# bottledspace/refraction-raytracing-dxr

Hardware: AMD Instinct MI355X
Metric: Mrays/s (primary+refracted) at 1920x1080, monkey.obj (higher is better)
Workload: dtype f32

## Files before the change

refraction_raytracing_dxr_amd/_build.py:

```python
import os
import shutil
import subprocess

PKG = os.path.dirname(os.path.abspath(__file__))
CSRC = os.path.join(PKG, "csrc")
LIB = os.path.join(PKG, "librrdxr.so")
DEMO = os.path.join(PKG, "rrdemo")

DEVICE_SOURCES = ["rr_bvh_build.hip", "rr_render_fused.hip", "rr_render_paths.hip", "rr_render_lds.hip", "rr_render_stream.hip",
                  "rr_query.hip", "rr_query_multi.hip", "rr_frame.hip", "rr_shade_rays.hip", "rr_render_samples.hip",
                  "rr_render_adaptive.hip", "rr_render_lens.hip", "rr_render_spectral.hip", "rr_render_materials.hip"]
HOST_SOURCES = ["rr_capi.cpp", "rr_capi_build.cpp", "rr_capi_dispatch.cpp", "rr_capi_orbit.cpp", "rr_capi_query.cpp", "rr_capi_comm.cpp",
                "rr_choice.cpp", "host/rr_host_camera.cpp", "host/rr_host_mesh.cpp", "host/rr_host_image.cpp", "host/rr_host_partition.cpp",
                "host/Mesh.cpp", "host/RefractionDemo.cpp"]
HEADERS = ["rr_types.h", "rr_context.h", "rr_choice.h", "rr_device.h", "rr_launch.h", "rr_render_common.h", "rr_render_materials.h", "host/Mesh.hpp", "host/RefractionDemo.hpp", "host/rr_host_lens.h",
           "../../include/rrdxr.h"]

COMMON = ["-O3", "-std=c++17", "-fPIC", "-ffp-contract=off", "-fno-fast-math", "-Wall", "-Wno-unused-function"]
DEVICE_FLAGS = ["--offload-arch=gfx950", "-fno-gpu-rdc"] + os.environ.get("RR_EXTRA_DEFINES", "").split()


def _hipcc():
    exe = shutil.which("hipcc") or "/opt/rocm/bin/hipcc"
    if not os.path.exists(exe):
        raise RuntimeError("hipcc not found: the HIP extension cannot be built")
    return exe


def _stale(target, deps):
    if not os.path.exists(target):
        return True
    t = os.path.getmtime(target)
    return any((not os.path.exists(d)) or os.path.getmtime(d) > t for d in deps)


def build(force=False, verbose=False):
    hipcc = _hipcc()
    srcs = [os.path.join(CSRC, s) for s in DEVICE_SOURCES + HOST_SOURCES]
    deps = srcs + [os.path.join(CSRC, h) for h in HEADERS] + [os.path.abspath(__file__)]
    objdir = os.path.join(PKG, "build")
    os.makedirs(objdir, exist_ok=True)
    stamp = os.path.join(objdir, "flags.txt")
    flags = " ".join(COMMON + DEVICE_FLAGS + DEVICE_SOURCES)
    if not os.path.exists(stamp) or open(stamp).read() != flags:
        force = True
    objs = []
    for s in srcs:
        o = os.path.join(objdir, os.path.basename(s) + ".o")
        objs.append(o)
        if force or _stale(o, [s] + deps[len(srcs):]):
            cmd = [hipcc, "-c", "-x", "hip", s, "-o", o] + COMMON + DEVICE_FLAGS
            if verbose:
                print(" ".join(cmd))
            subprocess.run(cmd, check=True)
    if force or _stale(LIB, objs):
        cmd = [hipcc, "-shared", "-o", LIB] + objs + ["--offload-arch=gfx950", "-fno-gpu-rdc"]
        if verbose:
            print(" ".join(cmd))
        subprocess.run(cmd, check=True)
    if force:
        with open(stamp, "w") as f:
            f.write(flags)
    demo_src = os.path.join(CSRC, "tools", "rrdemo.cpp")
    if force or _stale(DEMO, [demo_src, LIB]):
        cmd = [hipcc, demo_src, "-o", DEMO, "-O2", "-std=c++17", "-L" + PKG, "-lrrdxr", "-Wl,-rpath,$ORIGIN"]
        subprocess.run(cmd, check=True)
    return LIB


if __name__ == "__main__":
    print(build(force=False, verbose=True))
```

refraction_raytracing_dxr_amd/csrc/rr_capi.cpp:

```cpp
#include "rr_context.h"

#include <dlfcn.h>
#include <new>

static_assert(CHOICE_TILE == (uint32_t)TILE && CHOICE_STREAM_MAX_GEN == STREAM_MAX_GEN, "rr_choice.h mirrors rr_types.h");

static_assert(sizeof(rr_vertex) == 32, "Vertex stride (Mesh.cpp:45)");
static_assert(sizeof(rr_instance_desc) == 64, "D3D12_RAYTRACING_INSTANCE_DESC");
static_assert(sizeof(rr_scene_constants) == 80, "SceneConstants");
static_assert(sizeof(rr_ray) == sizeof(rr_ray_dev) && sizeof(rr_hit) == sizeof(rr_hit_dev), "ray/hit ABI");
static_assert(offsetof(rr_ray, instance_mask) == 36 && offsetof(rr_ray_dev, instance_mask) == 36, "rr_ray.instance_mask");

namespace {
struct Roctx {
    int (*push)(const char*) = nullptr;
    int (*pop)() = nullptr;
    Roctx()
    {
        for (const char* lib : { "librocprofiler-sdk-roctx.so", "libroctx64.so" }) {
            if (void* h = dlopen(lib, RTLD_LAZY | RTLD_LOCAL)) {
                push = reinterpret_cast<int (*)(const char*)>(dlsym(h, "roctxRangePushA"));
                pop = reinterpret_cast<int (*)()>(dlsym(h, "roctxRangePop"));
                if (push && pop) return;
                push = nullptr; pop = nullptr;
// ... 51 lines not shown

uint32_t scene_stack_need(const rr_context* ctx)
{
    uint32_t blas_max = 0;
    for (uint32_t i = 0; i < ctx->n_insts; ++i) {
        const MeshRes& m = ctx->meshes[(size_t)ctx->inst_host[i].blas];
        if (m.depth > blas_max) blas_max = m.depth;
    }
    return ctx->single_identity ? blas_max : blas_max + ctx->tlas_depth;
}

Tiles tile_counts(uint32_t W, uint32_t H, uint32_t rank, uint32_t world)
{
    const uint32_t tiles_x = (W + TILE - 1) / TILE, n_tiles = tiles_x * ((H + TILE - 1) / TILE);
    return { tiles_x, n_tiles, n_tiles > rank ? (n_tiles - rank + world - 1) / world : 0, (n_tiles + world - 1) / world };
}

int join_lane(rr_context* ctx, uint32_t lane)
{
    if (ctx->lane_busy[lane]) {
        RR_HIP(hipStreamWaitEvent(ctx->stream, ctx->lane_done[lane].get(), 0));
        ctx->lane_busy[lane] = false;
    }
    return RR_OK;
}

int join_lanes(rr_context* ctx)
{
    for (uint32_t l = 0; l < rr_context::MAX_LANES; ++l)
        if (int r = join_lane(ctx, l)) return r;
    return RR_OK;
}

rr_dispatch_params params_or_default(const rr_dispatch_params* params)
{
    rr_dispatch_params p;
    return params ? *params : (rr_default_dispatch_params(&p), p);
}
}

extern "C" {
uint32_t rr_abi_version(void) { return RRDXR_ABI_VERSION; }

void rr_default_dispatch_params(rr_dispatch_params* p)
{
    if (!p) return;
    p->max_refract = 5;
    p->max_reflect = 2;
    p->ior = 1.3f;
    p->tmin_primary = 0.0001f;
    p->tmax_primary = 100.0f;
    p->tmin_secondary = 0.001f;
    p->tmax_secondary = 1000.0f;
    p->flags = 0;
}

int rr_create(int device_ordinal, rr_context** out)
{
    if (!out) return RR_ERR_INVALID_ARGUMENT;
    *out = nullptr;
    int n = 0;
    if (hipGetDeviceCount(&n) != hipSuccess || n <= 0) return RR_ERR_NO_DEVICE;
    if (device_ordinal < 0 || device_ordinal >= n) return RR_ERR_INVALID_ARGUMENT;
    hipDeviceProp_t prop;
    if (hipGetDeviceProperties(&prop, device_ordinal) != hipSuccess) return RR_ERR_NO_DEVICE;
    if (strncmp(prop.gcnArchName, "gfx950", 6) != 0) return RR_ERR_NO_DEVICE;
    rr_context* ctx = new (std::nothrow) rr_context();
    if (!ctx) return RR_ERR_OUT_OF_MEMORY;
    ctx->device = device_ordinal;
    ctx->n_cus = prop.multiProcessorCount > 0 ? prop.multiProcessorCount : 256;
    if (hipSetDevice(device_ordinal) != hipSuccess || ctx->own_stream.create(hipStreamNonBlocking) != hipSuccess ||
        ctx->d_cnt.alloc(1) != hipSuccess || ctx->d_tickets.alloc((rr_context::MAX_LANES + 1) * LDS_TICKET_WORDS) != hipSuccess) {
        delete ctx;
        return RR_ERR_DEVICE;
    }
    ctx->stream = ctx->own_stream.get();
    (void)hipMemsetAsync(ctx->d_cnt.get(), 0, sizeof(CounterBlock), ctx->stream);
    (void)hipMemsetAsync(ctx->d_tickets.get(), 0, (rr_context::MAX_LANES + 1) * LDS_TICKET_WORDS * sizeof(uint32_t), ctx->stream);
    if (const char* e = getenv("RR_DEBUG_KERNEL"))
        ctx->dbg.kernel = !strcmp(e, "fused") ? 1 : !strcmp(e, "lds") ? 4 : !strcmp(e, "paths") ? 5 : !strcmp(e, "stream") ? 10 : 0;
    if (const char* e = getenv("RR_DEBUG_STACK")) ctx->dbg.stack = atoi(e);
    if (const char* e = getenv("RR_DEBUG_TICKET")) ctx->dbg_ticket_blocks = atoi(e);
    if (const char* e = getenv("RR_DEBUG_SHAPE")) ctx->dbg_shape = atoi(e);
    if (const char* e = getenv("RR_DEBUG_REFINE_GROUPS")) ctx->dbg_refine_groups = std::max(atoi(e), 0);
    if (const char* e = getenv("RR_DEBUG_TLAS32")) ctx->dbg.tlas32 = atoi(e) != 0;
    if (const char* e = getenv("RR_DEBUG_TILE_ORDER")) ctx->dbg_tile_order = atoi(e) != 0;
    if (const char* e = getenv("RR_DEBUG_ASYNC")) { unsigned l = 2, sh = 2; if (sscanf(e, "%u,%u", &l, &sh) == 2 && l >= 1 && sh >= 1) { ctx->dbg_async[0] = l; ctx->dbg_async[1] = sh; ctx->dbg_async_set = true; } }
    if (const char* e = getenv("RR_DEBUG_DIAG")) ctx->dbg_diag = e;
    if (const char* e = getenv("RR_DEBUG_GROUP_TRACE")) ctx->dbg_group_trace = atoi(e) != 0;
    *out = ctx;
    return RR_OK;
}

int rr_destroy(rr_context* ctx)
{
    if (!ctx) return RR_ERR_INVALID_ARGUMENT;
    (void)hipSetDevice(ctx->device);
    (void)hipStreamSynchronize(ctx->stream);
    for (const Stream& s : ctx->lane_stream) if (s.get()) (void)hipStreamSynchronize(s.get());
    delete ctx;
    return RR_OK;
}

const char* rr_last_error(const rr_context* ctx) { return ctx ? ctx->err.c_str() : "null context"; }

int rr_set_stream(rr_context* ctx, void* hip_stream)
{
    if (int r = use_device(ctx)) return r;
    RR_HIP(hipStreamSynchronize(ctx->stream));
    ctx->stream = (hipStream_t)hip_stream;
    return RR_OK;
}

int rr_reset_stream(rr_context* ctx)
{
    if (int r = use_device(ctx)) return r;
    RR_HIP(hipStreamSynchronize(ctx->stream));
    ctx->stream = ctx->own_stream.get();
    return RR_OK;
}

int rr_wait(rr_context* ctx)
{
    if (int r = use_device(ctx)) return r;
    if (int r = join_lanes(ctx)) return r;
    RR_HIP(hipStreamSynchronize(ctx->stream));
    return RR_OK;
}

int rr_set_frames_in_flight(rr_context* ctx, uint32_t n)
{
    if (int r = use_device(ctx)) return r;
    if (n == 0 || n > rr_context::MAX_LANES) return fail(ctx, RR_ERR_INVALID_ARGUMENT, "rr_set_frames_in_flight: 1..4");
    ctx->frames_in_flight = n;
    return RR_OK;
}

int rr_lane_join(rr_context* ctx, uint32_t lane)
{
    if (int r = use_device(ctx)) return r;
    if (lane >= rr_context::MAX_LANES) return fail(ctx, RR_ERR_INVALID_ARGUMENT, "rr_lane_join: lane out of range");
    return join_lane(ctx, lane);
}

int rr_upload_mesh(rr_context* ctx, const rr_vertex* verts, uint32_t n_verts, const uint32_t* indices, uint32_t n_indices,
                   uint32_t* mesh_id)
{
    if (int r = use_device(ctx)) return r;
    if (!verts || !indices || !mesh_id || n_verts == 0 || n_indices < 3 || n_indices % 3 != 0)
        return fail(ctx, RR_ERR_INVALID_ARGUMENT, "rr_upload_mesh: need >= 1 triangle, n_indices % 3 == 0");
    for (uint32_t i = 0; i < n_indices; ++i)
        if (indices[i] >= n_verts) return fail(ctx, RR_ERR_INVALID_ARGUMENT, "rr_upload_mesh: index out of range");
    if (rr_host_validate_positions(verts, n_verts, nullptr) != RR_OK)
        return fail(ctx, RR_ERR_INVALID_ARGUMENT, "rr_upload_mesh: non-finite or huge (> 1e18) vertex position");
    MeshRes m;
    m.n_verts = n_verts; m.n_idx = n_indices; m.n_tris = n_indices / 3;
    RR_HIP(m.d_verts.alloc((size_t)n_verts * 8));
    if (hipError_t e = m.d_idx.alloc(n_indices)) return fail(ctx, RR_ERR_OUT_OF_MEMORY, "hipMalloc(indices)", e);
    RR_HIP_MSG(hipMemcpyAsync(m.d_verts.get(), verts, (size_t)n_verts * sizeof(rr_vertex), hipMemcpyHostToDevice, ctx->stream), "mesh upload");
    RR_HIP_MSG(hipMemcpyAsync(m.d_idx.get(), indices, (size_t)n_indices * 4, hipMemcpyHostToDevice, ctx->stream), "mesh upload");
    RR_HIP_MSG(hipStreamSynchronize(ctx->stream), "mesh upload");
    ctx->meshes.push_back(std::move(m));
    *mesh_id = (uint32_t)ctx->meshes.size() - 1u;
    return RR_OK;
}

// ... 189 lines not shown
```

refraction_raytracing_dxr_amd/csrc/rr_capi_dispatch.cpp:

```cpp
#include "rr_context.h"

namespace {
int ensure_cams(rr_context* ctx, size_t n)
{
    return n <= ctx->d_cams.size() ? RR_OK : ctx->d_cams.grow(ctx, n < 64 ? 64 : n);
}

constexpr size_t STREAM_BUDGET_MAX = (size_t)48 << 30, STREAM_BUDGET_MIN = (size_t)1 << 30;
constexpr uint32_t STREAM_BLK = 1024;

size_t stream_budget(rr_context* ctx)
{
    if (ctx->strm_budget == 0) {
        size_t free_b = 0, total_b = 0;
        size_t b = STREAM_BUDGET_MAX;
        if (hipMemGetInfo(&free_b, &total_b) == hipSuccess) b = std::min(b, free_b / 6u);
        if (const char* e = getenv("RR_DEBUG_STREAM_BUDGET_GB")) { const long g = atol(e); if (g > 0 && g <= 200) b = (size_t)g << 30; }
        ctx->strm_budget = std::max(b, STREAM_BUDGET_MIN);
    }
    return ctx->strm_budget;
}

uint32_t lds_node_bytes(const MeshRes& m) { return m.n_nodes() * (uint32_t)sizeof(QNode); }

// ... 103 lines not shown
    o.want_f32 = (p.flags & RR_DISPATCH_FLOAT_OUTPUT) != 0;
    o.compact = ctx->tile_world > 1 || ext_tiles != nullptr;
    o.rgb8 = (p.flags & RR_DISPATCH_TILES_RGB8) != 0;
    if (o.rgb8 && !ext_tiles) return fail(ctx, RR_ERR_UNSUPPORTED, "dispatch: RGB8 tiles only exist in external tile buffers (rr_render_orbit_sharded)");
    o.slice_elems = o.compact ? (size_t)o.max_local * TILE * TILE * (o.rgb8 ? 3 : 4) / 4 : (size_t)width * height;
    o.stride = ext_tiles ? req.ext_stride_elems : o.slice_elems;
    if (ext_tiles && o.want_f32) return fail(ctx, RR_ERR_UNSUPPORTED, "dispatch: float output is not available for external tile buffers");
    o.out_base = ext_tiles ? 0 : o.slice_elems * req.out_slot_depth * req.out_slot;
    if (!ext_tiles)
        if (int r = ensure_frame_buffers(ctx, o.out_base + o.slice_elems * depth, o.want_f32)) return r;
    if (width != ctx->screen_w || height != ctx->screen_h) {
        RR_HIP(hipDeviceSynchronize());
        ctx->screen_w = ctx->screen_h = 0;
        RR_HIP(ctx->d_screen.alloc((size_t)width + height));
        RR_HIP(launch_screen_tables(ctx->d_screen.get(), width, height, ctx->stream));
        RR_HIP(hipStreamSynchronize(ctx->stream));
        ctx->screen_w = width; ctx->screen_h = height;
    }
    return RR_OK;
}

void set_rect_tiles(DispatchDev& a, uint32_t x0, uint32_t y0, uint32_t w, uint32_t h)
{
    a.rt_x0 = x0; a.rt_y0 = y0; a.rt_w = w; a.rt_h = h;
    a.rt_div_w = (uint32_t)(0x100000000ull / w) + 1u;
    a.rt_div_o = a.tiles_x > w ? (uint32_t)(0x100000000ull / (a.tiles_x - w)) + 1u : 0u;
}

void point_counters(DispatchDev& a, CounterBlock* c) { a.counters = c->counters; a.ray_shards = c->shards; a.error_flag = &c->error; }

DispatchDev make_dispatch(const rr_context* ctx, const DispatchRequest& req, const Layout& o)
{
    const uint32_t width = req.width, height = req.height, depth = req.depth;
    const rr_dispatch_params& p = req.params; const MeshOut* const mesh = req.mesh;
    DispatchDev a;
    memset(&a, 0, sizeof a);
    a.sx = ctx->d_screen.get(); a.sy = ctx->d_screen.get() + width;
    a.async_leaf_num = ctx->dbg_async[0]; a.async_shade_num = ctx->dbg_async[1];
    a.group_trace = ctx->dbg_group_trace ? 1u : 0u;
    uint32_t hr[4];
    (void)rr_host_screen_rect(ctx->scene_bounds, (p.flags & RR_DISPATCH_DEBUG_NO_CULL) ? nullptr : req.h_cams, depth, width, height, hr);
    a.hx0 = hr[0]; a.hy0 = hr[1]; a.hx1 = hr[2]; a.hy1 = hr[3];
    a.W = width; a.H = height; a.tiles_x = o.tiles_x; a.n_tiles = o.n_tiles;
    if (mesh) {
        a.mesh_part = 1u; a.n_mesh_local = o.n_mesh_local; a.n_rect_tiles = o.part.n_mesh_tiles; a.mesh_rounds = o.part.rank0_rounds;
        a.out_bg = mesh->bg; a.bg_stride = mesh->bg_stride_elems;
        if (o.part.rect_w) set_rect_tiles(a, o.part.rect_x0, o.part.rect_y0, o.part.rect_w, o.part.rect_h);
    } else if (ctx->dbg_tile_order && ctx->tile_world == 1 && o.n_tiles < 65536u && a.hx1 > a.hx0 && a.hy1 > a.hy0) {
        const uint32_t tiles_y = (height + TILE - 1) / TILE;
        const uint32_t x0 = a.hx0 / TILE, y0 = a.hy0 / TILE;
        const uint32_t x1 = std::min(o.tiles_x, (a.hx1 + TILE - 1) / TILE), y1 = std::min(tiles_y, (a.hy1 + TILE - 1) / TILE);
        if (x1 > x0 && y1 > y0 && (x1 - x0) * (y1 - y0) < o.n_tiles) set_rect_tiles(a, x0, y0, x1 - x0, y1 - y0);
    }
    a.cams = req.d_cams; a.n_frames = depth;
    a.blocks_per_frame = ((o.local + 7u) & ~7u) * 4u;
    a.frame_stride = o.stride;
    a.tile_rank = ctx->tile_rank; a.tile_world = ctx->tile_world; a.n_local_tiles = o.local;
    a.n_blocks = a.blocks_per_frame * depth;
    a.compact_out = o.compact ? (o.rgb8 ? 2u : 1u) : 0u;
    a.tonemap = (p.flags & RR_DISPATCH_TONEMAP_REINHARD) ? 1u : 0u;
    a.max_refract = p.max_refract; a.max_reflect = p.max_reflect;
    a.ior = p.ior; a.inv_ior = inv_ior_of(p.ior);
    a.tmin_p = p.tmin_primary; a.tmax_p = p.tmax_primary; a.tmin_s = p.tmin_secondary; a.tmax_s = p.tmax_secondary;
    a.out_rgba8 = req.ext_tiles ? req.ext_tiles : ctx->d_rgba8.get() + o.out_base;
    a.out_f32 = o.want_f32 ? ctx->d_f32.get() + o.out_base : nullptr;
    point_counters(a, ctx->d_cnt.get());
    return a;
}

struct Launch {
    SceneDev sc;
    DispatchDev a;
    uint32_t need;
    const rr_scene_constants* h_cams; const rr_dispatch_params* p;
    FusedVariant fused;
};

int ensure_lds_park(rr_context* ctx, uint32_t slot, int max_reflect)
{
    const size_t park_need = (size_t)ctx->n_cus * 32 * (max_reflect <= 2 ? 2u : 8u) * 8 * 64;
    return ctx->d_park[slot].size() < park_need ? ctx->d_park[slot].grow(ctx, park_need) : RR_OK;
}

int launch_lds(rr_context* ctx, const Launch& L, bool stats)
{
    const MeshRes& m0 = ctx->meshes[(size_t)ctx->inst_host[0].blas];
    LdsDispatch q;
    memset(&q, 0, sizeof q);
    const uint32_t slot = stream_slot(ctx);
    q.tickets = ctx->d_tickets.get() + (size_t)slot * LDS_TICKET_WORDS;
    q.park_slots = L.p->max_reflect <= 2 ? 2u : 8u;
    if (int r = ensure_lds_park(ctx, slot, L.p->max_reflect)) return r;
    q.park = ctx->d_park[slot].get();
    uint32_t rect[4];
    (void)rr_host_screen_rect(m0.bounds, ((ctx->dbg_ticket_blocks & 3) == 1 || (L.p->flags & RR_DISPATCH_DEBUG_NO_CULL)) ? nullptr : L.h_cams, L.a.n_frames,
                     L.a.W, L.a.H, rect);
    if ((ctx->dbg_ticket_blocks & 3) == 2) rect[2] = rect[0];
    q.n_queues = (ctx->dbg_ticket_blocks & 64) ? 64u : (ctx->dbg_ticket_blocks & 128) ? LDS_QUEUES : 8u;
    q.home_xcc = (ctx->dbg_ticket_blocks & 16) ? 0u : 1u;
    q.rx0 = rect[0]; q.ry0 = rect[1]; q.rx1 = rect[2]; q.ry1 = rect[3];
    q.node_bytes = lds_node_bytes(m0);
    q.stack_entries = L.need + 1;
    RR_HIP(launch_render_lds(L.sc, L.a, q, ctx->n_cus, stats, ctx->stream, ctx->dbg_shape));
    return RR_OK;
}

int launch_kernel(rr_context* ctx, const Launch& L, int kernel, bool stats)
{
    if (kernel == K_STREAM) return render_stream(ctx, L.sc, L.a, L.a.n_frames, (int)L.need, stats);
    if (kernel == K_LDS) return launch_lds(ctx, L, stats);
    if (kernel == K_PATHS) RR_HIP(launch_render_paths(L.sc, L.a, (int)L.need, stats, ctx->stream));
    else RR_HIP(launch_render_fused(L.sc, L.a, L.fused.stack, L.fused.pend, stats, ctx->stream, L.fused.stack16));
    return RR_OK;
}

int time_candidates(rr_context* ctx, Launch L, int cand_a, int cand_b, float ms[2])
{
    if (cand_b == K_STREAM) if (int r = ensure_stream_buffers(ctx, stream_plan(ctx, L.a, L.a.n_frames))) return r;
    if (cand_a == K_LDS || cand_b == K_LDS) if (int r = ensure_lds_park(ctx, stream_slot(ctx), L.p->max_reflect)) return r;
    for (Event& e : ctx->ch_ev) if (!e.get()) RR_HIP(e.create(hipEventDefault));
    if (!ctx->d_cnt_trial.get()) RR_HIP(ctx->d_cnt_trial.alloc(1));
    RR_HIP(hipDeviceSynchronize());
    RR_HIP(hipMemsetAsync(ctx->d_cnt_trial.get(), 0, sizeof(CounterBlock), ctx->stream));
    point_counters(L.a, ctx->d_cnt_trial.get());
    if (int r = launch_kernel(ctx, L, cand_a, false)) return r;
    for (int c = 0; c < 2; ++c) {
        RR_HIP(hipEventRecord(ctx->ch_ev[2 * c].get(), ctx->stream));
        if (int r = launch_kernel(ctx, L, c == 0 ? cand_a : cand_b, false)) return r;
        RR_HIP(hipEventRecord(ctx->ch_ev[2 * c + 1].get(), ctx->stream));
    }
    RR_HIP(hipEventSynchronize(ctx->ch_ev[3].get()));
    RR_HIP(hipEventElapsedTime(&ms[0], ctx->ch_ev[0].get(), ctx->ch_ev[1].get()));
    RR_HIP(hipEventElapsedTime(&ms[1], ctx->ch_ev[2].get(), ctx->ch_ev[3].get()));
    return RR_OK;
}

int choose_kernel(rr_context* ctx, const Launch& L, const KernelPick& pk, const LaunchFacts& lf, int& kernel)
{
    kernel = pk.kernel;
    if (pk.cls == CLS_NONE) return RR_OK;
    KernelChoice* const ch = ctx->ch[pk.cls].find(choice_key(L.a.W, L.a.H, *L.p, L.a.n_frames));
    if (measure_due(*ch, lf.rect_share, lf.no_cull)) {
        float ms[2] = { 0.0f, 0.0f };
        if (int r = time_candidates(ctx, L, pk.cand_a, pk.cand_b, ms)) return r;
        record_timings(*ch, ms[0], ms[1], lf.rect_share);
        if (getenv("RR_DEBUG_CHOICE"))
            fprintf(stderr, "[rr] kernel choice: depth %u candidate %d: default %.3f ms, candidate %.3f ms (%.3f)%s\n", L.a.n_frames, pk.cand_b, ms[0], ms[1],
                    ms[1] / ms[0], ch->choice == 2 ? " -> candidate" : ch->choice == 1 ? " -> default" : " (once more)");
    }
    kernel = chosen_kernel(pk, ch, lf.rect_share);
    return RR_OK;
}
}

namespace rr {
int ensure_frame_buffers(rr_context* ctx, size_t elems, bool want_f32)
{
    if (elems > ctx->d_rgba8.size())
        if (int r = ctx->d_rgba8.grow(ctx, elems)) return r;
    if (want_f32 && elems > ctx->d_f32.size()) return ctx->d_f32.grow(ctx, elems);
    return RR_OK;
}

int check_shading_params(rr_context* ctx, const char* who, const rr_dispatch_params& p)
{
    const std::string w(who);
    if (p.max_refract < 0 || p.max_refract > 65535 || p.max_reflect < 0)
        return fail(ctx, RR_ERR_INVALID_ARGUMENT, (w + ": negative bounce limit").c_str());
    if (p.max_reflect > 8) return fail(ctx, RR_ERR_UNSUPPORTED, (w + ": max_reflect > 8 (parked-ray registers)").c_str());
    if (!(p.ior > 0.0f)) return fail(ctx, RR_ERR_INVALID_ARGUMENT, (w + ": ior must be > 0").c_str());
    return RR_OK;
}

SceneFacts scene_facts(const rr_context* ctx)
{
    SceneFacts s = { ctx->single_identity, scene_stack_need(ctx), 0, ctx->n_pool_nodes, ctx->n_pool_tris + ctx->n_insts, false };
    if (ctx->single_identity && !ctx->inst_host.empty()) {
        const MeshRes& m0 = ctx->meshes[(size_t)ctx->inst_host[0].blas];
        s.blas_tris = m0.n_tris;
        s.lds_fits = ctx->dbg.stack == 0 && m0.n_tris < 32768u && lds_kernel_shape(lds_node_bytes(m0), s.need + 1, nullptr, ctx->dbg_shape) >= 0;
    }
    return s;
}

LaunchPick pick_launch(const rr_context* ctx, const DispatchRequest& req, const uint32_t rect[4], bool compact)
{
// ... 163 lines not shown
```

refraction_raytracing_dxr_amd/csrc/rr_context.h:

```cpp
#pragma once
#include "../../include/rrdxr.h"

#include <hip/hip_runtime.h>

#include <algorithm>
#include <cmath>
#include <cstdio>
#include <cstdlib>
#include <cstring>
#include <string>
#include <vector>

#include "rr_choice.h"
#include "rr_launch.h"

namespace rr {

struct Range {
    explicit Range(const char* name);
    ~Range();
};

template <class T, bool Pinned = false> class Buf {
public:
// ... 79 lines not shown
    DevBuf<uint8_t>  pending;
};

}

using namespace rr;

struct rr_context {
    int device = 0;
    int n_cus = 256;
    Stream      own_stream;
    hipStream_t stream = nullptr;
    std::string err;

    std::vector<MeshRes> meshes;

    DevBuf<float4> d_env;
    int env_w = 0, env_h = 0;

    std::vector<rr_instance_desc> inst_host;
    DevBuf<InstDev> d_insts;
    DevBuf<BvhNode> d_pool_nodes;
    DevBuf<QNode>   d_pool_qnodes;
    QGrid    scene_grid = { { 0, 0, 0 }, { 1, 1, 1 } };
    DevBuf<TriRec>  d_pool_tris;
    DevBuf<NrmRec>  d_pool_nrms;
    uint32_t n_pool_tris = 0, n_pool_nodes = 0;
    uint32_t n_insts = 0, tlas_depth = 0;
    bool tlas_built = false;
    bool single_identity = false;
    float scene_scale = 1.0f;
    float scene_bounds[6] = { 0, 0, 0, 0, 0, 0 };
    std::vector<uint32_t> pool_node_off, pool_tri_off;
    std::vector<uint64_t> pool_version;
    DevBuf<int32_t>  d_tlas_links;
    DevBuf<uint32_t> d_tlas_visit;
    bool tlas_refittable = false;

    DevBuf<float> d_screen;
    uint32_t screen_w = 0, screen_h = 0;

    rr_scene_constants cam;
    bool cam_set = false;
    DevBuf<CamDev> d_cams;
    static constexpr int CAM_SLOTS = 4;
    HostBuf<CamDev> h_cams[CAM_SLOTS];
    Event      h_cams_ev[CAM_SLOTS];
    bool       h_cams_busy[CAM_SLOTS] = {};
    uint32_t   h_cams_next = 0;

    uint32_t tile_rank = 0, tile_world = 1;

    static constexpr uint32_t MAX_LANES = 4;
    Stream      lane_stream[MAX_LANES];
    Event       lane_fork[MAX_LANES], lane_done[MAX_LANES];
    DevBuf<CamDev> lane_cams[MAX_LANES];
    bool        lane_busy[MAX_LANES] = {};
    uint32_t    frames_in_flight = 2;
    size_t      frame_base = 0;

    uint32_t W = 0, H = 0, frame_world = 0, frame_depth = 1;
    DevBuf<uint32_t> d_rgba8;
    DevBuf<float4>   d_f32;
    DevBuf<uint32_t> d_assembled;
    bool      have_f32 = false, have_frame = false, have_assembled = false;
    uint64_t  last_pixels = 0;
    uint64_t  accum_pixels = 0;
    bool      last_stats = false;

    DevBuf<CounterBlock> d_cnt;
    DevBuf<CounterBlock> d_cnt_trial;
    DevBuf<uint32_t> d_park[MAX_LANES + 1];
    char       last_kernel_name[96] = "";
    uint32_t   last_kernel = 0;
    DevBuf<uint32_t> d_tickets;

    DebugFacts dbg = { 0, 0, false };
    int  dbg_ticket_blocks = 0;
    bool dbg_group_trace = true;
    bool dbg_async_set = false;
    uint32_t dbg_async[2] = { 2, 2 };
    bool dbg_tile_order = true;
    int  dbg_shape = 0;
    int  dbg_refine_groups = 0;
    std::string dbg_diag;

    Event ev_begin, ev_end;
    std::vector<Event> kev;
    uint32_t kev_used = 0;

    StreamSet strm[MAX_LANES + 1];
    size_t    strm_budget = 0;
    ChoiceClass ch[3];
    Event      ch_ev[4];

    DevBuf<rr_ray_dev> d_rays;
    DevBuf<rr_hit_dev> d_hits;
    DevBuf<uint32_t>   d_counts;
    DevBuf<float4>     d_out_f32;
    DevBuf<uint32_t>   d_out_rgba8, d_out_n;
    DevBuf<uint32_t>   d_adaptive_taken;
    DevBuf<float4>     d_adaptive_ws;
    DevBuf<MatDev>     d_mats;
    uint32_t n_mats = 0, max_material = 0;
};

namespace rr {

int fail(rr_context* ctx, int code, const char* what, hipError_t e = hipSuccess);

#define RR_HIP(call)                                                                      \
    do {                                                                                  \
        hipError_t e_ = (call);                                                           \
        if (e_ != hipSuccess) return fail(ctx, e_ == hipErrorOutOfMemory ? RR_ERR_OUT_OF_MEMORY : RR_ERR_DEVICE, #call, e_); \
    } while (0)

#define RR_HIP_MSG(call, what)                                                            \
    do {                                                                                  \
        hipError_t e_ = (call);                                                           \
        if (e_ != hipSuccess) return fail(ctx, RR_ERR_DEVICE, what, e_);                  \
    } while (0)

template <class T, bool Pinned> int Buf<T, Pinned>::grow(rr_context* ctx, size_t n)
{
    RR_HIP(hipStreamSynchronize(ctx->stream));
    RR_HIP(alloc(n));
    return RR_OK;
}

int use_device(rr_context* ctx);
void fill_scene(const rr_context* ctx, SceneDev& sc);
uint32_t inst0_mask(const rr_context* ctx);
uint32_t scene_stack_need(const rr_context* ctx);
rr_dispatch_params params_or_default(const rr_dispatch_params* params);
struct Tiles { uint32_t tiles_x, n_tiles, local, max_local; };
Tiles tile_counts(uint32_t W, uint32_t H, uint32_t rank, uint32_t world);
int join_lane(rr_context* ctx, uint32_t lane);
int join_lanes(rr_context* ctx);

struct MeshOut { const rr_mesh_partition* part; uint32_t* bg; size_t bg_stride_elems; };

struct DispatchRequest {
    uint32_t width = 0, height = 0, depth = 1;
    const CamDev* d_cams = nullptr; const rr_scene_constants* h_cams = nullptr;
    rr_dispatch_params params = {};
    uint32_t* ext_tiles = nullptr; size_t ext_stride_elems = 0;
    bool keep_counters = false;
    uint32_t out_slot = 0, out_slot_depth = 0;
    const MeshOut* mesh = nullptr;
};
int dispatch_impl(rr_context* ctx, const DispatchRequest& req);
int upload_cams(rr_context* ctx, const rr_scene_constants* c, size_t n);
int ensure_frame_buffers(rr_context* ctx, size_t elems, bool want_f32);
int check_shading_params(rr_context* ctx, const char* who, const rr_dispatch_params& p);
int check_error_flag(rr_context* ctx, const char* what);
SceneFacts scene_facts(const rr_context* ctx);
struct LaunchPick { SceneFacts sf; LaunchFacts lf; KernelPick pk; };
LaunchPick pick_launch(const rr_context* ctx, const DispatchRequest& req, const uint32_t rect[4], bool compact);

}
```

refraction_raytracing_dxr_amd/csrc/rr_launch.h:

```cpp
#pragma once
#include <hip/hip_runtime.h>
#include "rr_types.h"
#include "host/rr_host_lens.h"

namespace rr {

struct alignas(16) rr_ray_dev { float origin[3]; float tmin; float dir[3]; float tmax; uint32_t flags; uint32_t instance_mask; uint32_t pad[2]; };
struct rr_hit_dev { float t, u, v; uint32_t prim, inst, hit; };
static_assert(sizeof(rr_ray_dev) == 48 && sizeof(rr_hit_dev) == 24, "ABI layout");

hipError_t launch_render_fused(const SceneDev& sc, const DispatchDev& a, int stack, int pend, bool stats, hipStream_t s,
                               bool stack16 = false);
const char* last_render_kernel_name();
void set_render_kernel_name(const char* fmt, ...) __attribute__((format(printf, 1, 2)));
hipError_t launch_render_paths(const SceneDev& sc, const DispatchDev& a, int stack, bool stats, hipStream_t s);
int lds_kernel_shape(uint32_t node_bytes, uint32_t stack_entries, size_t* lds_bytes, int min_shape = 0);
hipError_t launch_render_lds(const SceneDev& sc, const DispatchDev& a, LdsDispatch q, int n_cus, bool stats, hipStream_t s, int min_shape = 0);
hipError_t launch_render_stream(const SceneDev& sc, const DispatchDev& a, const StreamDev& s, int stack, uint32_t n_wg, bool stats, hipStream_t st);
hipError_t launch_env_lookup(const SceneDev& sc, const float* dirs, uint32_t n, float* rgb, hipStream_t s);
hipError_t launch_trace_rays(const SceneDev& sc, const rr_ray_dev* rays, uint32_t n, rr_hit_dev* hits, uint32_t* err,
                             int stack, hipStream_t s);
hipError_t launch_query_rays(const SceneDev& sc, const rr_ray_dev* rays, uint32_t n, rr_hit_dev* hits, uint32_t inst0_mask, int stack,
                             hipStream_t s);
constexpr uint32_t RR_QUERY_MULTI_MAX_K = 16;
hipError_t launch_query_multi(const SceneDev& sc, const rr_ray_dev* rays, uint32_t n, uint32_t k, rr_hit_dev* hits, uint32_t* counts,
                              uint32_t inst0_mask, int stack, hipStream_t s);
hipError_t launch_shade_rays(const SceneDev& sc, const DispatchDev& a, const rr_ray_dev* rays, uint32_t n, float4* f32, uint32_t* rgba8,
                             uint32_t* n_rays, int stack, int pend, bool stack16, hipStream_t s);
struct SampleOffsets { static constexpr uint32_t MAX = 64; float v[2 * MAX]; };
hipError_t launch_render_samples(const SceneDev& sc, const DispatchDev& a, const CamDev& cam, const SampleOffsets& off, uint32_t n_samples,
                                 float4* f32, uint32_t* rgba8, uint32_t* n_rays, int stack, int pend, bool stack16, hipStream_t s);
hipError_t launch_render_lens(const SceneDev& sc, const DispatchDev& a, const CamDev& cam, const SampleOffsets& off, const SampleOffsets& loff,
                              const LensDev& lens, uint32_t n_samples, float4* f32, uint32_t* rgba8, uint32_t* n_rays, int stack, int pend,
                              bool stack16, hipStream_t s);
struct BandTable { static constexpr uint32_t MAX = SampleOffsets::MAX; float ior[MAX]; float inv_ior[MAX]; float weight[MAX][3]; };
hipError_t launch_render_spectral(const SceneDev& sc, const DispatchDev& a, const CamDev& cam, const SampleOffsets& off, const BandTable& bands,
                                  uint32_t n_samples, float4* f32, uint32_t* rgba8, uint32_t* n_rays, int stack, int pend, bool stack16,
                                  hipStream_t s);
hipError_t launch_shade_rays_mat(const SceneDev& sc, const DispatchDev& a, const MatDev* mats, uint32_t mat0, const rr_ray_dev* rays, uint32_t n,
                                 float4* f32, uint32_t* rgba8, uint32_t* n_rays, int stack, int pend, bool stack16, hipStream_t s);
hipError_t launch_render_materials(const SceneDev& sc, const DispatchDev& a, const CamDev& cam, const SampleOffsets& off, const MatDev* mats,
                                   uint32_t mat0, uint32_t n_samples, float4* f32, uint32_t* rgba8, uint32_t* n_rays, int stack, int pend,
                                   bool stack16, hipStream_t s);
struct AdaptiveWorkspace {
    float4* rec; uint32_t* cnt; uint32_t* list; unsigned long long* masks; uint32_t* base; uint32_t* total;
    uint64_t bytes;
    AdaptiveWorkspace(void* p, uint32_t W, uint32_t H)
    {
        const uint64_t n = (uint64_t)W * H, nb = (uint64_t)((W + 7u) / 8u) * ((H + 7u) / 8u);
        const uint64_t o_cnt = 16u * n, o_list = o_cnt + 4u * n, o_masks = (o_list + 4u * n + 15u) & ~(uint64_t)15u, o_base = o_masks + 8u * nb;
        const uintptr_t c = reinterpret_cast<uintptr_t>(p);
        rec = static_cast<float4*>(p); cnt = reinterpret_cast<uint32_t*>(c + o_cnt); list = reinterpret_cast<uint32_t*>(c + o_list);
        masks = reinterpret_cast<unsigned long long*>(c + o_masks); base = reinterpret_cast<uint32_t*>(c + o_base); total = base + nb;
        bytes = (o_base + 4u * (nb + 1u) + 15u) & ~(uint64_t)15u;
    }
};
hipError_t launch_render_adaptive(const SceneDev& sc, const DispatchDev& a, const CamDev& cam, const SampleOffsets& off, uint32_t n_base,
                                  uint32_t n_max, float threshold, const AdaptiveWorkspace& ws, float4* f32, uint32_t* rgba8, uint32_t* n_rays,
                                  uint32_t* n_taken, int stack, int pend, bool stack16, uint32_t refine_groups, hipStream_t s);
hipError_t launch_screen_tables(float* out, uint32_t W, uint32_t H, hipStream_t s);
hipError_t launch_assemble_tiles(const uint32_t* gathered, uint32_t* frame, uint32_t W, uint32_t H, uint32_t tiles_x,
                                 uint32_t n_tiles, uint32_t world, uint32_t max_tiles, hipStream_t s);
hipError_t launch_assemble_frames(const uint32_t* gathered, uint32_t* frames, uint32_t W, uint32_t H, uint32_t tiles_x,
                                  uint32_t n_tiles, uint32_t world, size_t rank_stride, size_t frame_stride,
                                  size_t out_stride, uint32_t n_frames, hipStream_t s);
hipError_t launch_assemble_frames_rgb8(const uint8_t* gathered, uint32_t* frames, uint32_t W, uint32_t H, uint32_t tiles_x, uint32_t n_tiles,
                                       uint32_t world, size_t rank_stride_b, size_t frame_stride_b, size_t out_stride, uint32_t n_frames,
                                       hipStream_t s);
hipError_t launch_assemble_frames_mesh_rgb8(const uint8_t* gathered, const uint8_t* bg, uint32_t* frames, uint32_t W, uint32_t H, const MeshPartDev& mp,
                                            size_t rank_stride_b, size_t frame_stride_b, size_t bg_stride_b, size_t out_stride, uint32_t n_frames, hipStream_t s);

struct BuildBuffers {
    uint32_t n;
    uint32_t n_pad;
    float*   prim_box;
    unsigned long long* keys;
    int32_t* parent;
    int32_t* child;
    float*   node_box;
    uint32_t* visit;
    uint32_t* scene_box;
    uint32_t* depth;
    uint32_t* ploc;
    BvhNode* nodes;
    uint32_t leaf_ref_prim;
    uint32_t leaf_base;
};

hipError_t launch_tri_setup(const void* verts, const uint32_t* idx, uint32_t n_tris, const BuildBuffers& b, hipStream_t s);
hipError_t launch_lbvh(const BuildBuffers& b, hipStream_t s);
constexpr uint32_t PLOC_MAX_PRIMS = 32768;
hipError_t launch_ploc(const BuildBuffers& b, hipStream_t s);
hipError_t launch_pack_tris(const void* verts, const uint32_t* idx, const BuildBuffers& b, TriRec* tris, NrmRec* nrms,
                            hipStream_t s);
hipError_t launch_inst_setup(const InstDev* insts, const float* blas_bounds, uint32_t n, const BuildBuffers& b, hipStream_t s);
hipError_t launch_quantize_nodes(QNode* dst, const BvhNode* src, uint32_t n_nodes, const QGrid& g, uint32_t node_off, uint32_t tri_off,
                                 hipStream_t s);
hipError_t launch_keep_links(const BuildBuffers& b, int32_t* links, hipStream_t s);
hipError_t launch_refit_blas(const void* verts, const uint32_t* idx, uint32_t n_tris, TriRec* tris, NrmRec* nrms, BvhNode* nodes,
                             const int32_t* links, uint32_t* visit, uint32_t* scene_box, hipStream_t s);
// ... 7 lines not shown
```

refraction_raytracing_dxr_amd/csrc/rr_render_lds.hip:

```cpp
#include <hip/hip_runtime.h>
#include "rr_render_common.h"

namespace rr {

__device__ __forceinline__ BlockPos lds_tile_block(const DispatchDev& a, const LdsDispatch& q, uint32_t u, uint32_t j)
{
    BlockPos p;
    const uint32_t tile = a.n_frames == 1u ? u : __umulhi(u, q.div_frames);
    p.frame = u - tile * a.n_frames;
    p.tile_local = tile;
    p.tile_ok = tile < a.n_local_tiles;
    p.bg = false;
    const uint32_t ty = a.tiles_x == 1u ? tile : __umulhi(tile, q.div_tiles_x), tx = tile - ty * a.tiles_x;
    p.px0 = (j & 3u) * 8u; p.py0 = (j >> 2) * 8u;
    p.x0 = tx * TILE + p.px0; p.y0 = ty * TILE + p.py0;
    return p;
}

__device__ __forceinline__ BlockPos lds_rect_block(const DispatchDev& a, const LdsDispatch& q, uint32_t u, uint32_t j)
{
    BlockPos p;
    const uint32_t strip = a.n_frames == 1u ? u : __umulhi(u, q.div_frames), per_row = q.rect_bw >> 2;
    p.frame = u - strip * a.n_frames;
    const uint32_t row = per_row == 1u ? strip : __umulhi(strip, q.div_per_row), col = strip - row * per_row;
// ... 82 lines not shown
                    if (t < n_tickets) { u = qi + NQ * t; drew = true; break; }
                }
                ++tried;
                qi = qi + 1u == NQ ? 0u : qi + 1u;
            }
            if (!drew) { ++phase; qi = home; tried = 0u; continue; }
            if (phase == 0u) {
                if (lane == 0) wg_share[wave] = ((unsigned long long)(u + 1u) << 32) | 1ull;
                bp = lds_rect_block(a, q, u, 0u);
                have = true;
            } else {
                if (lane == 0) wg_share[wave] = ((unsigned long long)((u + 1u) | 0x80000000u) << 32) | 1ull;
                bp = lds_tile_block(a, q, u, 0u);
                have = bp.tile_ok && !in_rect(bp);
            }
        }
        if (!have) break;
        st.blocks += 1u;
        const unsigned long long dr0 = DIAG ? __builtin_amdgcn_s_memtime() : 0ull;
        const uint32_t dI0 = DIAG ? diag_tr[wave] : 0u, dL0 = DIAG ? diag_tr[16 + wave] : 0u, dS0 = DIAG ? diag_tr[32 + wave] : 0u;
        const uint32_t x = bp.x0 + lx, y = bp.y0 + ly;
        const bool may_hit = bp.x0 + 8u > a.hx0 && bp.x0 < a.hx1 && bp.y0 + 8u > a.hy0 && bp.y0 < a.hy1;
        if (STATS && !may_hit) st.bg_blocks += 1u;
        if (x < a.W && y < a.H) {
            const CamDev& cb = a.cams[bp.frame];
            st.pixels += 1;
            const f3 acc = render_pixel<STATS, false, DIAG, E, LdsNodes>(sc, a, cb, x, y, may_hit, stk, ns, park, st, Diag{ DIAG ? &diag_tr[wave] : nullptr, 16 });
            const size_t o = a.compact_out == 0u ? (size_t)y * a.W + x
                                                : (size_t)bp.tile_local * (TILE * TILE) + (bp.py0 + ly) * TILE + (bp.px0 + lx);
            store_pixel(a, a.out_rgba8 + (size_t)bp.frame * a.frame_stride,
                        a.out_f32 ? a.out_f32 + (size_t)bp.frame * a.frame_stride : nullptr, o, acc);
        }
        if (DIAG) {
            const unsigned long long dt = __builtin_amdgcn_s_memtime() - dr0;
            diag_render += dt; diag_n += 1ull << 32;
            if (dt > diag_worst) {
                diag_worst = dt;
                diag_worst_trips = (unsigned long long)(diag_tr[wave] - dI0) | ((unsigned long long)(diag_tr[16 + wave] - dL0) << 20) |
                                   ((unsigned long long)(diag_tr[32 + wave] - dS0) << 40);
            }
        }
    }
    if (DIAG && lane == 0) {
        unsigned long long* d = a.diag + (size_t)(blockIdx.x * NW + wave) * 8;
        d[0] = diag_wait; d[1] = diag_render; d[2] = diag_n; d[3] = __builtin_amdgcn_s_memtime() - diag_t0;
        d[4] = diag_worst; d[5] = diag_worst_trips; d[6] = diag_t1 - diag_t0; d[7] = diag_tr[wave] | ((unsigned long long)diag_tr[16 + wave] << 32);
    }
    flush_stats<STATS>(a, st, blockIdx.x * NW + wave, lane);
    if (lane == 0) {
        const uint32_t w_arrived = atomicAdd(&wg_arrived, 1u);
        if (w_arrived + 1u == (uint32_t)NW) {
            const uint32_t arrived = atomicAdd(&q.tickets[2u * LDS_QUEUES * 16u], 1u);
            if (arrived + 1u == gridDim.x) {
                for (uint32_t k = 0; k <= 2u * LDS_QUEUES; ++k) atomicExch(&q.tickets[k * 16u], 0u);
            }
        }
    }
}

constexpr struct { int nw, wgs; } LDS_SHAPES[] = { { 12, 2 }, { 16, 2 }, { 16, 1 } };
static size_t lds_shape_bytes(int i, uint32_t node_bytes, uint32_t stack_entries) { return (size_t)node_bytes + (size_t)LDS_SHAPES[i].nw * stack_entries * 64 * sizeof(uint16_t); }

int lds_kernel_shape(uint32_t node_bytes, uint32_t stack_entries, size_t* lds_bytes, int min_shape)
{
    for (int i = min_shape < 0 ? 0 : min_shape; i < 3; ++i) {
        const size_t need = lds_shape_bytes(i, node_bytes, stack_entries);
        if (need <= (size_t)(160 * 1024) / LDS_SHAPES[i].wgs - 512) { if (lds_bytes) *lds_bytes = need; return i; }
        if (min_shape <= 0) break;
    }
    return -1;
}

template <int SHAPE, bool STATS, bool DIAG = false>
static hipError_t launch_lds_nw(const SceneDev& sc, const DispatchDev& a, const LdsDispatch& q, int n_cus, hipStream_t s)
{
    constexpr int NW = LDS_SHAPES[SHAPE].nw, WGS = LDS_SHAPES[SHAPE].wgs;
    static const hipError_t attr = hipFuncSetAttribute(reinterpret_cast<const void*>(&k_render_lds<NW, WGS, STATS, DIAG>), hipFuncAttributeMaxDynamicSharedMemorySize, 159 * 1024);
    if (attr != hipSuccess) return attr;
    if (!DIAG) set_render_kernel_name("k_render_lds<%d, %d, %s, false>", NW, WGS, STATS ? "true" : "false");
    hipLaunchKernelGGL((k_render_lds<NW, WGS, STATS, DIAG>), dim3((uint32_t)n_cus * WGS), dim3(NW * 64), lds_shape_bytes(SHAPE, q.node_bytes, q.stack_entries), s, sc, a, q);
    return hipGetLastError();
}

hipError_t launch_render_lds(const SceneDev& sc, const DispatchDev& a, LdsDispatch q, int n_cus, bool stats, hipStream_t s, int min_shape)
{
    if (a.n_blocks == 0) return hipSuccess;
    const int shape = lds_kernel_shape(q.node_bytes, q.stack_entries, nullptr, min_shape);
    if (shape < 0) return hipErrorInvalidValue;
    {
        const uint32_t grid = (uint32_t)n_cus * (uint32_t)LDS_SHAPES[shape].wgs;
        if (q.n_queues > grid) q.n_queues = grid;
        if (q.n_queues > LDS_QUEUES) q.n_queues = LDS_QUEUES;
        if (q.n_queues < 1u) q.n_queues = 1u;
    }
    q.p2_tickets = a.n_local_tiles * a.n_frames;
    if (q.rx1 > q.rx0 && q.ry1 > q.ry0) {
        q.rx0 &= ~31u;
        q.rx1 = (q.rx1 + 31u) & ~31u;
    }
    const bool rect = q.rx1 > q.rx0 && q.ry1 > q.ry0;
    q.rect_bw = rect ? (q.rx1 - q.rx0) / 8u : 0u;
    q.p1_tickets = !rect ? 0u : (q.rect_bw / 4u) * ((q.ry1 - q.ry0) / 8u) * a.n_frames;
    if ((uint64_t)q.p2_tickets * a.n_frames >= 0xffffffffull || (uint64_t)q.p1_tickets * a.n_frames >= 0xffffffffull) return hipErrorInvalidValue;
    q.div_frames = (uint32_t)(0x100000000ull / a.n_frames) + 1u;
    q.div_tiles_x = (uint32_t)(0x100000000ull / a.tiles_x) + 1u;
    q.div_per_row = rect ? (uint32_t)(0x100000000ull / (q.rect_bw / 4u)) + 1u : 0u;
    static_assert(sizeof LDS_SHAPES / sizeof LDS_SHAPES[0] == 3, "lds_kernel_shape and the rungs below");
    if (a.diag) return launch_lds_nw<0, false, true>(sc, a, q, n_cus, s);
    if (shape == 0) return stats ? launch_lds_nw<0, true>(sc, a, q, n_cus, s) : launch_lds_nw<0, false>(sc, a, q, n_cus, s);
    if (shape == 1) return stats ? launch_lds_nw<1, true>(sc, a, q, n_cus, s) : launch_lds_nw<1, false>(sc, a, q, n_cus, s);
    return stats ? launch_lds_nw<2, true>(sc, a, q, n_cus, s) : launch_lds_nw<2, false>(sc, a, q, n_cus, s);
}

}
```

Before: 30190.

## Route tiles outside geometry bounds to a dedicated background-only kernel

Adds a lightweight env-lookup kernel for tiles outside the projected geometry rectangle. By default the LDS traversal kernel gets no phase-2 tile tickets and processes only the expanded hit rectangle. The remaining pixels get camera-ray environment lookups without BVH traversal or LDS setup. Correctness relies on the hit rectangle conservatively covering all geometry, and it adds a second kernel launch.

```diff
diff --git a/refraction_raytracing_dxr_amd/_build.py b/refraction_raytracing_dxr_amd/_build.py
--- a/refraction_raytracing_dxr_amd/_build.py
+++ b/refraction_raytracing_dxr_amd/_build.py
@@ -7,7 +7,7 @@
 LIB = os.path.join(PKG, "librrdxr.so")
 DEMO = os.path.join(PKG, "rrdemo")
 
-DEVICE_SOURCES = ["rr_bvh_build.hip", "rr_render_fused.hip", "rr_render_paths.hip", "rr_render_lds.hip", "rr_render_stream.hip",
+DEVICE_SOURCES = ["rr_bvh_build.hip", "rr_render_fused.hip", "rr_render_paths.hip", "rr_render_lds.hip", "rr_render_background.hip", "rr_render_stream.hip",
                   "rr_query.hip", "rr_query_multi.hip", "rr_frame.hip", "rr_shade_rays.hip", "rr_render_samples.hip",
                   "rr_render_adaptive.hip", "rr_render_lens.hip", "rr_render_spectral.hip", "rr_render_materials.hip"]
 HOST_SOURCES = ["rr_capi.cpp", "rr_capi_build.cpp", "rr_capi_dispatch.cpp", "rr_capi_orbit.cpp", "rr_capi_query.cpp", "rr_capi_comm.cpp",
diff --git a/refraction_raytracing_dxr_amd/csrc/rr_capi.cpp b/refraction_raytracing_dxr_amd/csrc/rr_capi.cpp
--- a/refraction_raytracing_dxr_amd/csrc/rr_capi.cpp
+++ b/refraction_raytracing_dxr_amd/csrc/rr_capi.cpp
@@ -157,6 +157,7 @@
     if (const char* e = getenv("RR_DEBUG_STACK")) ctx->dbg.stack = atoi(e);
     if (const char* e = getenv("RR_DEBUG_TICKET")) ctx->dbg_ticket_blocks = atoi(e);
     if (const char* e = getenv("RR_DEBUG_SHAPE")) ctx->dbg_shape = atoi(e);
+    if (const char* e = getenv("RR_DEBUG_BG_SPLIT")) { const int v = atoi(e); if (v >= 0 && v <= 16) ctx->dbg_bg_split = v; }
     if (const char* e = getenv("RR_DEBUG_REFINE_GROUPS")) ctx->dbg_refine_groups = std::max(atoi(e), 0);
     if (const char* e = getenv("RR_DEBUG_TLAS32")) ctx->dbg.tlas32 = atoi(e) != 0;
     if (const char* e = getenv("RR_DEBUG_TILE_ORDER")) ctx->dbg_tile_order = atoi(e) != 0;
diff --git a/refraction_raytracing_dxr_amd/csrc/rr_capi_dispatch.cpp b/refraction_raytracing_dxr_amd/csrc/rr_capi_dispatch.cpp
--- a/refraction_raytracing_dxr_amd/csrc/rr_capi_dispatch.cpp
+++ b/refraction_raytracing_dxr_amd/csrc/rr_capi_dispatch.cpp
@@ -209,6 +209,8 @@
     return ctx->d_park[slot].size() < park_need ? ctx->d_park[slot].grow(ctx, park_need) : RR_OK;
 }
 
+uint32_t lds_default_bg_split(uint32_t ) { return 0u; }
+
 int launch_lds(rr_context* ctx, const Launch& L, bool stats)
 {
     const MeshRes& m0 = ctx->meshes[(size_t)ctx->inst_host[0].blas];
@@ -225,10 +227,29 @@
     if ((ctx->dbg_ticket_blocks & 3) == 2) rect[2] = rect[0];
     q.n_queues = (ctx->dbg_ticket_blocks & 64) ? 64u : (ctx->dbg_ticket_blocks & 128) ? LDS_QUEUES : 8u;
     q.home_xcc = (ctx->dbg_ticket_blocks & 16) ? 0u : 1u;
+    const uint32_t n_tiles = L.a.n_local_tiles;
+    uint32_t keep = n_tiles;
+    if (!L.a.diag && (ctx->dbg_ticket_blocks & 3) != 2) {
+        const uint32_t sixteenths = ctx->dbg_bg_split >= 0 ? (uint32_t)ctx->dbg_bg_split : lds_default_bg_split(L.a.n_frames);
+        keep = (uint32_t)(((uint64_t)n_tiles * sixteenths + 15u) / 16u);
+        if (L.a.hx1 > L.a.hx0 && L.a.hy1 > L.a.hy0) {
+            if (rect[2] > rect[0] && rect[3] > rect[1]) {
+                rect[0] = std::min(rect[0], L.a.hx0); rect[1] = std::min(rect[1], L.a.hy0);
+                rect[2] = std::max(rect[2], L.a.hx1); rect[3] = std::max(rect[3], L.a.hy1);
+            } else {
+                rect[0] = L.a.hx0; rect[1] = L.a.hy0; rect[2] = L.a.hx1; rect[3] = L.a.hy1;
+            }
+        }
+    }
+    if (rect[2] > rect[0] && rect[3] > rect[1]) {
+        rect[0] &= ~31u;
+        rect[2] = (rect[2] + 31u) & ~31u;
+    }
     q.rx0 = rect[0]; q.ry0 = rect[1]; q.rx1 = rect[2]; q.ry1 = rect[3];
     q.node_bytes = lds_node_bytes(m0);
     q.stack_entries = L.need + 1;
-    RR_HIP(launch_render_lds(L.sc, L.a, q, ctx->n_cus, stats, ctx->stream, ctx->dbg_shape));
+    RR_HIP(launch_render_lds(L.sc, L.a, q, ctx->n_cus, stats, ctx->stream, ctx->dbg_shape, keep));
+    if (keep < n_tiles) RR_HIP(launch_render_background(L.sc, L.a, rect, keep, ctx->stream, stats));
     return RR_OK;
 }
 
diff --git a/refraction_raytracing_dxr_amd/csrc/rr_context.h b/refraction_raytracing_dxr_amd/csrc/rr_context.h
--- a/refraction_raytracing_dxr_amd/csrc/rr_context.h
+++ b/refraction_raytracing_dxr_amd/csrc/rr_context.h
@@ -185,6 +185,7 @@
     uint32_t dbg_async[2] = { 2, 2 };
     bool dbg_tile_order = true;
     int  dbg_shape = 0;
+    int  dbg_bg_split = -1;
     int  dbg_refine_groups = 0;
     std::string dbg_diag;
 
diff --git a/refraction_raytracing_dxr_amd/csrc/rr_launch.h b/refraction_raytracing_dxr_amd/csrc/rr_launch.h
--- a/refraction_raytracing_dxr_amd/csrc/rr_launch.h
+++ b/refraction_raytracing_dxr_amd/csrc/rr_launch.h
@@ -15,7 +15,9 @@
 void set_render_kernel_name(const char* fmt, ...) __attribute__((format(printf, 1, 2)));
 hipError_t launch_render_paths(const SceneDev& sc, const DispatchDev& a, int stack, bool stats, hipStream_t s);
 int lds_kernel_shape(uint32_t node_bytes, uint32_t stack_entries, size_t* lds_bytes, int min_shape = 0);
-hipError_t launch_render_lds(const SceneDev& sc, const DispatchDev& a, LdsDispatch q, int n_cus, bool stats, hipStream_t s, int min_shape = 0);
+hipError_t launch_render_lds(const SceneDev& sc, const DispatchDev& a, LdsDispatch q, int n_cus, bool stats, hipStream_t s, int min_shape = 0,
+                             uint32_t keep_tiles = 0xffffffffu);
+hipError_t launch_render_background(const SceneDev& sc, const DispatchDev& a, const uint32_t rect[4], uint32_t first_tile, hipStream_t s, bool stats);
 hipError_t launch_render_stream(const SceneDev& sc, const DispatchDev& a, const StreamDev& s, int stack, uint32_t n_wg, bool stats, hipStream_t st);
 hipError_t launch_env_lookup(const SceneDev& sc, const float* dirs, uint32_t n, float* rgb, hipStream_t s);
 hipError_t launch_trace_rays(const SceneDev& sc, const rr_ray_dev* rays, uint32_t n, rr_hit_dev* hits, uint32_t* err,
diff --git a/refraction_raytracing_dxr_amd/csrc/rr_render_background.hip b/refraction_raytracing_dxr_amd/csrc/rr_render_background.hip
--- /dev/null
+++ b/refraction_raytracing_dxr_amd/csrc/rr_render_background.hip
@@ -0,0 +1,97 @@
+#include <hip/hip_runtime.h>
+#include "rr_render_common.h"
+
+namespace rr {
+
+struct BgTiles {
+    uint32_t rx0, ry0, rx1, ry1;
+    uint32_t first_tile, n_units;
+    uint32_t div_frames, div_tiles_x;
+};
+
+template <bool STATS>
+__global__ __launch_bounds__(256, 8) void k_background(SceneDev sc, DispatchDev a, BgTiles b)
+{
+    const uint32_t wave = __builtin_amdgcn_readfirstlane(threadIdx.x >> 6), lane = threadIdx.x & 63u;
+    const uint32_t u = blockIdx.x * 4u + wave;
+    LaneStats st;
+    stats_clock_begin<STATS>(st);
+    if (u < b.n_units) {
+        const uint32_t t = a.n_frames == 1u ? u : __umulhi(u, b.div_frames), frame = u - t * a.n_frames, tile = b.first_tile + t;
+        const uint32_t ty = a.tiles_x == 1u ? tile : __umulhi(tile, b.div_tiles_x), tx = tile - ty * a.tiles_x;
+        const uint32_t x0 = tx * TILE, y0 = ty * TILE;
+        const bool x_in = x0 >= b.rx0 && x0 < b.rx1;
+        uint32_t skip = 0u;
+        for (uint32_t r = 0; r < 4u; ++r) if (x_in && y0 + 8u * r >= b.ry0 && y0 + 8u * r < b.ry1) skip |= 1u << r;
+        if (skip != 0xfu) {
+            {
+                const uint32_t cols = a.W > x0 ? (a.W - x0 + 7u) / 8u : 0u, cols_in = cols < 4u ? cols : 4u;
+                uint32_t passes = 0u;
+                for (uint32_t r = 0; r < 4u; ++r)
+                    if (!(skip >> r & 1u)) { st.blocks += 4u; if (y0 + 8u * r < a.H) passes += cols_in; }
+                if (STATS) { st.bg_blocks = st.blocks; if (lane == 0) st.passes = passes; }
+            }
+            float M[12];
+#pragma unroll
+            for (int i = 0; i < 12; ++i) M[i] = a.cams[frame].M[i];
+            const uint32_t col = lane & 31u, x = x0 + col, half = lane >> 5;
+            const bool x_ok = x < a.W;
+            const float sx = a.sx[x_ok ? x : a.W - 1u];
+            uint32_t* const out = a.out_rgba8 + (size_t)frame * a.frame_stride;
+            float4* const out_f = a.out_f32 ? a.out_f32 + (size_t)frame * a.frame_stride : nullptr;
+            f3 e = mk3(0.0f, 0.0f, 0.0f);
+            size_t o = 0;
+            bool stored = false;
+            for (uint32_t r = 0; r < 4u; ++r) {
+                if (skip >> r & 1u) continue;
+                float sy[4];
+#pragma unroll
+                for (uint32_t k = 0; k < 4u; ++k) { const uint32_t y = y0 + 8u * r + 2u * k + half; sy[k] = a.sy[y < a.H ? y : a.H - 1u]; }
+#pragma unroll
+                for (uint32_t k = 0; k < 4u; ++k) {
+                    const uint32_t row = 8u * r + 2u * k + half, y = y0 + row;
+                    const bool ok = x_ok && y < a.H;
+                    const f3 e1 = env_lookup(sc, camera_ray_dir(M, sx, sy[k]));
+                    if (ok) { st.pixels += 1u; st.rays += 1u; if (STATS) st.miss += 1u; }
+                    if (stored) store_pixel(a, out, out_f, o, mk3(fmaf(1.0f, e.x, 0.0f), fmaf(1.0f, e.y, 0.0f), fmaf(1.0f, e.z, 0.0f)));
+                    e = e1; stored = ok;
+                    o = a.compact_out == 0u ? (size_t)y * a.W + x : (size_t)tile * (TILE * TILE) + row * TILE + col;
+                }
+            }
+            if (stored) store_pixel(a, out, out_f, o, mk3(fmaf(1.0f, e.x, 0.0f), fmaf(1.0f, e.y, 0.0f), fmaf(1.0f, e.z, 0.0f)));
+        }
+    }
+    flush_stats<STATS>(a, st, u, lane);
+}
+
+hipError_t launch_render_background(const SceneDev& sc, const DispatchDev& a, const uint32_t rect[4], uint32_t first_tile, hipStream_t s, bool stats)
+{
+    if (first_tile >= a.n_local_tiles || a.n_frames == 0u) return hipSuccess;
+    if ((rect[0] | rect[2]) & 31u || (rect[1] | rect[3]) & 7u) return hipErrorInvalidValue;
+    const bool have_rect = rect[2] > rect[0] && rect[3] > rect[1];
+    const uint32_t n = a.n_local_tiles, tiles_x = a.tiles_x;
+    if ((uint64_t)n * a.n_frames * a.n_frames >= 0xffffffffull) return hipErrorInvalidValue;
+    if (have_rect) {
+        const uint32_t ix0 = rect[0] / TILE, ix1 = rect[2] / TILE < tiles_x ? rect[2] / TILE : tiles_x;
+        const uint32_t iy0 = (rect[1] + TILE - 1u) / TILE, iy1 = rect[3] / TILE;
+        auto inside_below = [&](uint32_t k) -> uint64_t {
+            if (ix1 <= ix0 || iy1 <= iy0) return 0;
+            const uint32_t row = k / tiles_x, c = k - row * tiles_x;
+            const uint32_t full = row < iy0 ? 0u : (row < iy1 ? row : iy1) - iy0;
+            const uint32_t part = row >= iy0 && row < iy1 ? (c < ix0 ? 0u : (c < ix1 ? c : ix1) - ix0) : 0u;
+            return (uint64_t)full * (ix1 - ix0) + part;
+        };
+        if (inside_below(n) - inside_below(first_tile) == (uint64_t)(n - first_tile)) return hipSuccess;
+    }
+    BgTiles b;
+    b.rx0 = rect[0]; b.ry0 = rect[1]; b.rx1 = have_rect ? rect[2] : rect[0]; b.ry1 = rect[3];
+    b.first_tile = first_tile; b.n_units = (n - first_tile) * a.n_frames;
+    b.div_frames = (uint32_t)(0x100000000ull / a.n_frames) + 1u;
+    b.div_tiles_x = (uint32_t)(0x100000000ull / tiles_x) + 1u;
+    const dim3 grid((b.n_units + 3u) / 4u);
+    if (stats) hipLaunchKernelGGL((k_background<true>), grid, dim3(256), 0, s, sc, a, b);
+    else hipLaunchKernelGGL((k_background<false>), grid, dim3(256), 0, s, sc, a, b);
+    return hipGetLastError();
+}
+
+}
diff --git a/refraction_raytracing_dxr_amd/csrc/rr_render_lds.hip b/refraction_raytracing_dxr_amd/csrc/rr_render_lds.hip
--- a/refraction_raytracing_dxr_amd/csrc/rr_render_lds.hip
+++ b/refraction_raytracing_dxr_amd/csrc/rr_render_lds.hip
@@ -188,7 +188,8 @@
     return hipGetLastError();
 }
 
-hipError_t launch_render_lds(const SceneDev& sc, const DispatchDev& a, LdsDispatch q, int n_cus, bool stats, hipStream_t s, int min_shape)
+hipError_t launch_render_lds(const SceneDev& sc, const DispatchDev& a, LdsDispatch q, int n_cus, bool stats, hipStream_t s, int min_shape,
+                             uint32_t keep_tiles)
 {
     if (a.n_blocks == 0) return hipSuccess;
     const int shape = lds_kernel_shape(q.node_bytes, q.stack_entries, nullptr, min_shape);
@@ -199,7 +200,7 @@
         if (q.n_queues > LDS_QUEUES) q.n_queues = LDS_QUEUES;
         if (q.n_queues < 1u) q.n_queues = 1u;
     }
-    q.p2_tickets = a.n_local_tiles * a.n_frames;
+    q.p2_tickets = (keep_tiles < a.n_local_tiles ? keep_tiles : a.n_local_tiles) * a.n_frames;
     if (q.rx1 > q.rx0 && q.ry1 > q.ry0) {
         q.rx0 &= ~31u;
         q.rx1 = (q.rx1 + 31u) & ~31u;
@@ -207,7 +208,7 @@
     const bool rect = q.rx1 > q.rx0 && q.ry1 > q.ry0;
     q.rect_bw = rect ? (q.rx1 - q.rx0) / 8u : 0u;
     q.p1_tickets = !rect ? 0u : (q.rect_bw / 4u) * ((q.ry1 - q.ry0) / 8u) * a.n_frames;
-    if ((uint64_t)q.p2_tickets * a.n_frames >= 0xffffffffull || (uint64_t)q.p1_tickets * a.n_frames >= 0xffffffffull) return hipErrorInvalidValue;
+    if ((uint64_t)a.n_local_tiles * a.n_frames * a.n_frames >= 0xffffffffull || (uint64_t)q.p1_tickets * a.n_frames >= 0xffffffffull) return hipErrorInvalidValue;
     q.div_frames = (uint32_t)(0x100000000ull / a.n_frames) + 1u;
     q.div_tiles_x = (uint32_t)(0x100000000ull / a.tiles_x) + 1u;
     q.div_per_row = rect ? (uint32_t)(0x100000000ull / (q.rect_bw / 4u)) + 1u : 0u;
```

Result: no change. 30050 (-0.5%).
